# adobe-research/DiffusionHandles

Measured on AMD Instinct MI355X. Metric: guided-denoise steps/sec at 512x512 (SD2-depth), higher is better.
Workload: dtype f16

## Files before the change

### diffusionhandles_amd/_lib.py

```python
import ctypes
import os

import torch

_HERE = os.path.dirname(os.path.abspath(__file__))
LIB_PATH = os.environ.get("DIFFHANDLES_LIB") or os.path.join(_HERE, "libdiffhandles_hip.so")
_LIB = None

c_p = ctypes.c_void_p
c_i = ctypes.c_int
c_f = ctypes.c_float
c_d = ctypes.c_double
c_sz = ctypes.c_size_t


class UNetConfig(ctypes.Structure):
    _fields_ = [("in_channels", c_i), ("out_channels", c_i), ("n_levels", c_i),
                ("block_out_channels", c_i * 4), ("layers_per_block", c_i), ("heads", c_i * 4),
                ("cross_attention_dim", c_i), ("norm_groups", c_i), ("sample_size", c_i),
                ("text_len", c_i), ("max_batch", c_i), ("dtype", c_i), ("max_diff_batch", c_i)]


class VAEConfig(ctypes.Structure):
    _fields_ = [("latent_channels", c_i), ("out_channels", c_i), ("block_out_channels", c_i * 4),
# ... 11 lines not shown
    "dh_device_count": (c_i, []),
    "dh_reproject_workspace_bytes": (c_i, [c_i, c_i, c_i, ctypes.POINTER(c_sz)]),
    "dh_fg_pixel_list": (c_i, [c_p, c_i, c_p, c_p, c_p, c_sz, c_p]),
    "dh_reproject_edits": (c_i, [c_p, c_p, c_p, c_i, c_i, c_p, c_p, c_f, c_f, c_d, c_d, c_i,
                                 ctypes.POINTER(c_d), c_p, c_p, c_p, c_p, c_p, c_p, c_p, c_p, c_p, c_p, c_sz, c_p]),
    "dh_unproject": (c_i, [c_p, c_i, c_p, c_p, c_f, c_f, c_p, c_p]),
    "dh_masked_centroid": (c_i, [c_p, c_p, c_i, c_i, c_p, c_p, c_f, c_f, c_p, c_p]),
    "dh_laplacian_blend_workspace_bytes": (c_i, [c_i, ctypes.POINTER(c_sz)]),
    "dh_laplacian_blend": (c_i, [c_p, c_p, c_p, c_i, c_i, c_p, c_p, c_p, c_sz, c_p]),
    "dh_cells_workspace_bytes": (c_i, [c_i, c_i, ctypes.POINTER(c_sz)]),
    "dh_cells_from_correspondences": (c_i, [c_p, c_i, c_i, c_i, c_i, c_p, c_p, c_p, c_p, c_p, c_sz, c_p]),
    "dh_energy_workspace_bytes": (c_i, [c_i, c_i, c_i, ctypes.POINTER(c_sz)]),
    "dh_energy_fwd_bwd": (c_i, [c_p, c_p, c_i, c_i, c_i, c_i, c_i, c_p, c_i, c_p, c_i, c_p, c_i, c_p, c_i,
                                c_f, c_f, c_i, c_i, c_i, c_f, c_p, c_p, c_i, c_p, c_sz, c_p]),
    "dh_mesh_workspace_bytes": (c_i, [c_i, ctypes.POINTER(c_sz)]),
    "dh_mesh_reproject": (c_i, [c_p, c_p, c_p, c_i, c_p, c_p, c_f, c_f, c_p, c_p, c_f, c_p, c_p, c_p, c_p, c_p, c_p,
                                c_sz, c_p]),
    "dh_energy_plan_bytes": (c_i, [c_i, c_i, ctypes.POINTER(c_sz)]),
    "dh_energy_plan_build": (c_i, [c_p, c_i, c_p, c_i, c_i, c_p, c_sz, c_p]),
    "dh_energy_planned_workspace_bytes": (c_i, [c_i, c_i, ctypes.POINTER(c_sz)]),
    "dh_energy_fwd_bwd_planned": (c_i, [c_p, c_p, c_i, c_i, c_i, c_p, c_sz, c_i, c_p, c_i, c_p, c_i, c_f, c_f, c_f,
                                        c_p, c_p, c_i, c_p, c_sz, c_p]),
    "dh_unet_create": (c_i, [ctypes.POINTER(UNetConfig), ctypes.POINTER(c_p)]),
    "dh_unet_create_shared": (c_i, [c_p, c_i, c_p, ctypes.POINTER(c_p)]),
    "dh_unet_destroy": (None, [c_p]),
    "dh_unet_num_params": (c_i, [c_p]),
    "dh_unet_param_info": (c_i, [c_p, c_i, ctypes.POINTER(ctypes.c_char_p), ctypes.POINTER(c_i),
                                 ctypes.POINTER(ctypes.c_int64)]),
    "dh_unet_load_param": (c_i, [c_p, c_i, c_p, c_p]),
    "dh_unet_weight_bytes": (c_sz, [c_p]),
    "dh_unet_workspace_bytes": (c_sz, [c_p]),
    "dh_unet_forward": (c_i, [c_p, c_p, c_f, c_p, c_i, c_i, c_p, ctypes.POINTER(c_p), c_p]),
    "dh_unet_backward": (c_i, [c_p, ctypes.POINTER(c_p), c_p, c_p, c_p, c_p]),
    "dh_unet_set_text_key": (c_i, [c_p, ctypes.c_ulonglong]),
    "dh_unet_stats": (c_i, [c_p, ctypes.POINTER(c_d), ctypes.POINTER(c_d), ctypes.POINTER(ctypes.c_int64)]),
    "dh_vae_decoder_create": (c_i, [c_p, ctypes.POINTER(c_p)]),
    "dh_vae_decoder_destroy": (None, [c_p]),
    "dh_vae_decoder_num_params": (c_i, [c_p]),
    "dh_vae_decoder_param_info": (c_i, [c_p, c_i, ctypes.POINTER(ctypes.c_char_p), ctypes.POINTER(c_i),
                                        ctypes.POINTER(ctypes.c_int64)]),
    "dh_vae_decoder_load_param": (c_i, [c_p, c_i, c_p, c_p]),
    "dh_vae_decoder_bytes": (c_sz, [c_p]),
    "dh_vae_decoder_decode": (c_i, [c_p, c_p, c_i, c_p, c_p]),
    "dh_vae_encoder_create": (c_i, [c_p, ctypes.POINTER(c_p)]),
    "dh_vae_encoder_encode": (c_i, [c_p, c_p, c_i, c_p, c_p]),
    "dh_text_encoder_create": (c_i, [c_p, ctypes.POINTER(c_p)]),
    "dh_text_encoder_destroy": (None, [c_p]),
    "dh_text_encoder_num_params": (c_i, [c_p]),
    "dh_text_encoder_param_info": (c_i, [c_p, c_i, ctypes.POINTER(ctypes.c_char_p), ctypes.POINTER(c_i),
                                         ctypes.POINTER(ctypes.c_int64)]),
    "dh_text_encoder_load_param": (c_i, [c_p, c_i, c_p, c_p]),
    "dh_text_encoder_bytes": (c_sz, [c_p]),
    "dh_text_encoder_encode": (c_i, [c_p, c_p, c_i, c_i, c_p, c_p]),
    "dh_gemm_profile_begin": (c_i, []),
    "dh_gemm_profile_end": (c_i, [ctypes.POINTER(c_d), ctypes.POINTER(ctypes.c_int64), ctypes.POINTER(c_d)]),
    "dh_gemm_profile_bytes": (c_i, [ctypes.POINTER(c_d)]),
    "dh_ddim_cfg_step": (c_i, [c_p, c_p, c_p, c_p, c_f, c_f, c_f, c_i, c_p]),
    "dh_latent_update": (c_i, [c_p, c_p, c_p, c_f, c_f, c_i, c_p]),
    "dh_adam_step": (c_i, [c_p, c_p, c_p, c_p, c_f, c_f, c_f, c_f, c_i, c_i, c_p]),
    "dh_mse_fwd_bwd": (c_i, [c_p, c_p, c_i, c_p, c_p, c_p]),
    "dh_latent_update_strided": (c_i, [c_p, c_p, c_p, c_i, c_i, c_f, c_f, c_i, c_p]),
    "dh_pack_sample": (c_i, [c_p, c_p, c_i, c_i, c_p, c_i, c_i, c_i, c_i, c_p]),
    "dh_unet_io_ptr": (c_i, [c_p, c_i, c_i, ctypes.POINTER(c_p), ctypes.POINTER(c_sz)]),
    "dh_mse_cotangent": (c_i, [c_p, c_p, c_i, c_f, c_f, c_p, c_p, c_p, c_p]),
    "dh_adam_step_scaled": (c_i, [c_p, c_p, c_p, c_p, c_p, c_f, c_f, c_f, c_f, c_i, c_i, c_p]),
    "dh_mse_cotangent_batch": (c_i, [c_p, c_p, c_i, c_i, c_f, c_f, c_d, c_p, c_p, c_p, c_p, c_p, c_p]),
    "dh_adam_step_scaled_batch": (c_i, [c_p, c_p, c_p, c_p, c_p, c_p, c_f, c_f, c_f, c_f, c_i, c_i, c_i, c_p]),
}

c_l = ctypes.c_long
DEBUG_SIGNATURES = {
    "dh_dbg_gemm": (c_i, [c_i, c_p, c_l, c_p, c_i, c_i, c_i, c_i, c_i, c_i, c_i, c_i, c_i, c_i, c_i, c_p, c_p, c_i, c_i,
                          c_p, c_l, c_p, c_l, c_i, c_p, c_sz, c_p]),
    "dh_dbg_gemm_groupnorm": (c_i, [c_i, c_p, c_l, c_p, c_i, c_i, c_i, c_i, c_i, c_i, c_i, c_p, c_p, c_p, c_sz, c_i, c_i, c_p, c_p, c_f, c_i,
                                    c_p, c_p, c_p, ctypes.POINTER(c_i), c_p]),
    "dh_dbg_gemm_groupnorm_bwd": (c_i, [c_i, c_p, c_l, c_p, c_i, c_i, c_i, c_i, c_i, c_i, c_i, c_p, c_p, c_sz, c_i, c_i, c_p, c_p, c_p, c_p, c_i,
                                        c_p, c_p, ctypes.POINTER(c_i), c_p]),
    "dh_dbg_gemm_groupnorm_res": (c_i, [c_i, c_p, c_l, c_p, c_i, c_i, c_i, c_i, c_i, c_i, c_i, c_p, c_p, c_l, c_p, c_p, c_sz, c_i, c_i, c_p, c_p,
                                    c_f, c_i, c_p, c_p, c_p, ctypes.POINTER(c_i), c_p]),
    "dh_dbg_gemm_groupnorm_bwd_res": (c_i, [c_i, c_p, c_l, c_p, c_i, c_i, c_i, c_i, c_i, c_i, c_i, c_p, c_l, c_p, c_p, c_sz, c_i, c_i, c_p, c_p, c_p,
                                        c_p, c_i, c_p, c_p, ctypes.POINTER(c_i), c_p]),
    "dh_dbg_concat_groupnorm": (c_i, [c_i, c_p, c_i, c_p, c_i, c_p, c_i, c_i, c_i, c_p, c_p, c_f, c_i, c_p, c_p, c_p, c_p]),
    "dh_dbg_gemm_last_tile": (c_i, [ctypes.POINTER(c_i)]),
    "dh_dbg_unet_concat_ops": (c_i, [ctypes.POINTER(UNetConfig), ctypes.POINTER(c_i), c_i, ctypes.POINTER(c_i)]),
    "dh_dbg_gemm_lnfold": (c_i, [c_i, c_p, c_l, c_p, c_i, c_i, c_i, c_p, c_p, c_p, c_f, c_p, c_l, c_p]),
    "dh_dbg_gemm_glu": (c_i, [c_i, c_i, c_p, c_l, c_p, c_i, c_i, c_i, c_p, c_p, c_p, c_p, c_p, c_p]),
    "dh_dbg_gemm_family": (c_i, [c_i]),
    "dh_dbg_gemm_stage": (c_i, [c_i]),
    "dh_dbg_gemm_pp_variant": (c_i, [c_i, c_p]),
    "dh_dbg_gemm_pp_ablate": (c_i, [c_i]),
    "dh_dbg_gemm_pp_persist": (c_i, [c_i]),
    "dh_dbg_gemm_pp_glu": (c_i, [c_i]),
    "dh_dbg_gemm_pp_plan": (c_i, [c_i, c_i, c_i, c_i, c_i, c_i, c_sz, ctypes.POINTER(c_i), ctypes.POINTER(c_i), ctypes.POINTER(c_i)]),
    "dh_dbg_touch_tiled": (c_i, [c_sz, c_p]),
    "dh_dbg_groupnorm": (c_i, [c_i, c_p, c_p, c_p, c_p, c_p, c_p, c_p, c_p, c_i, c_i, c_i, c_i, c_f, c_i, c_i, c_p]),
    "dh_dbg_layernorm": (c_i, [c_i, c_p, c_p, c_p, c_p, c_p, c_p, c_p, c_p, c_i, c_i, c_f, c_p]),
    "dh_dbg_geglu": (c_i, [c_i, c_p, c_p, c_p, c_p, c_i, c_i, c_p]),
    "dh_dbg_attention": (c_i, [c_i, c_p, c_l, c_p, c_p, c_l, c_p, c_l, c_p, c_p, c_p, c_p, c_p, c_p, c_i, c_i, c_i, c_i, c_p]),
    "dh_dbg_attention_bwd_pair": (c_i, [c_i, c_p, c_l, c_p, c_p, c_l, c_p, c_l, c_p, c_p, c_p, c_p, c_p, c_p, c_i, c_i, c_i, c_i, c_p, c_p]),
    "dh_dbg_pool2x2": (c_i, [c_i, c_p, c_p, c_i, c_i, c_i, c_i, c_i, c_p]),
    "dh_dbg_ellipse_offsets": (c_i, [c_i, ctypes.POINTER(ctypes.c_int32), c_i, ctypes.POINTER(c_i)]),
    "dh_dbg_lane_ops": (c_i, [c_p, c_p, c_p, c_p]),
}


def lib():
    global _LIB
    if _LIB is None:
        if not os.path.exists(LIB_PATH):
            raise RuntimeError(
                f"native HIP library not found at {LIB_PATH}; build it with "
                "`python -c 'import __graft_entry__ as g; g.build()'` (there is no CPU fallback)")
        handle = ctypes.CDLL(LIB_PATH)
        missing = []
        for name, (res, args) in list(SIGNATURES.items()) + list(DEBUG_SIGNATURES.items()):
            try:
                fn = getattr(handle, name)
            except AttributeError:
                missing.append(name)
                continue
            fn.restype = res
            fn.argtypes = args
        handle.dh_missing_symbols = missing
        for env, fn in (("DH_GEMM_FAMILY", "dh_dbg_gemm_family"), ("DH_PP_GLU", "dh_dbg_gemm_pp_glu"),
                        ("DH_PP_PERSIST", "dh_dbg_gemm_pp_persist"), ("DH_GEMM_STAGE", "dh_dbg_gemm_stage")):
            if os.environ.get(env) and fn not in missing:
                getattr(handle, fn)(int(os.environ[env]))
        _LIB = handle
    return _LIB


def check(rc, what=""):
    if rc != 0:
        raise RuntimeError(f"{what} failed ({rc}): {lib().dh_last_error().decode()}")


def require_gpu(t=None):
    if not torch.cuda.is_available():
        raise RuntimeError("diffusionhandles_amd needs a HIP device (MI355X); there is no CPU fallback")
    if t is not None and not t.is_cuda:
        raise RuntimeError("expected a device tensor")


def ptr(t):
    return c_p(t.data_ptr()) if t is not None else c_p(0)


def stream_ptr():
    return c_p(torch.cuda.current_stream().cuda_stream)


DTYPE_CODE = {torch.float16: 0, torch.bfloat16: 1, torch.float32: 2}
CODE_DTYPE = {v: k for k, v in DTYPE_CODE.items()}
```

### diffusionhandles_amd/csrc/gemm.hip

```cpp
#include <stdlib.h>

#include <vector>

#include <hip/hip_ext.h>

#include "gemm_k.h"

namespace dh {

struct GemmProf {
  bool on = false;
  std::vector<hipEvent_t> ev;
  size_t used = 0;
  double flops = 0;
  double bytes = 0;
  hipEvent_t e0 = nullptr, e1 = nullptr;
};
static GemmProf g_prof;
static int g_buf_stage = 1;
static int g_pp_force = 0;
struct GemmTileReport {
  int bm, bn, kg, stages, mw, splits, pp, gn_epi, reduce_gn;
};
static thread_local GemmTileReport g_last_tile;
#ifdef DH_TUNING
static unsigned long long* g_gemm_ts = nullptr;
#endif
bool gemm_profiling_on() { return g_prof.on; }

constexpr int BK = 64;
#ifdef DH_EXP_SETPRIO
#define DH_PRIO(x) __builtin_amdgcn_s_setprio(x)
#else
#define DH_PRIO(x) do { } while (0)
#endif


template <class T>
__device__ __forceinline__ uint2 epilogue_pack(const GemmK& p, int m, int n, float v0, float v1, float v2, float v3,
                                               bool have_r, uint2 rpre, bool have_b, float4 bpre) {
  float v[4] = {v0, v1, v2, v3};
  if (p.bias) {
    float4 b = bpre;
    if (!have_b) b = *reinterpret_cast<const float4*>(p.bias + n);
    v[0] += b.x; v[1] += b.y; v[2] += b.z; v[3] += b.w;
  }
  if (p.rowvec) {
    const float4 b = *reinterpret_cast<const float4*>(p.rowvec + (size_t)div_small(m, p.inv_rows_per_batch) * p.rowvec_ld + n);
    v[0] += b.x; v[1] += b.y; v[2] += b.z; v[3] += b.w;
  }
  if (p.act_silu) {
#pragma unroll
    for (int i = 0; i < 4; ++i) v[i] = v[i] / (1.f + __expf(-v[i]));
  }
  typedef T T4 __attribute__((ext_vector_type(4)));
  if (p.R) {
    const T* r = reinterpret_cast<const T*>(p.R) + (size_t)m * p.ldr + n;
    uint2 raw = rpre;
    if (!have_r) raw = *reinterpret_cast<const uint2*>(r);
    const T4 rv = __builtin_bit_cast(T4, raw);
#pragma unroll
    for (int i = 0; i < 4; ++i) v[i] += to_f32<T>(rv[i]);
  }
  T4 o;
#pragma unroll
  for (int i = 0; i < 4; ++i) o[i] = from_f32<T>(v[i]);
  return __builtin_bit_cast(uint2, o);
}
template <class T>
__device__ __forceinline__ void epilogue_store(const GemmK& p, int m, int n, float v0, float v1, float v2, float v3,
                                               bool have_r = false, uint2 rpre = make_uint2(0, 0), bool have_b = false,
                                               float4 bpre = make_float4(0.f, 0.f, 0.f, 0.f)) {
  *reinterpret_cast<uint2*>(reinterpret_cast<T*>(p.C) + (size_t)m * p.ldc + n) =
      epilogue_pack<T>(p, m, n, v0, v1, v2, v3, have_r, rpre, have_b, bpre);
}

template <class T>
__device__ __forceinline__ float epilogue_scalar(const GemmK& p, int m, int n, float v) {
  if (p.bias) v += p.bias[n];
  if (p.rowvec) v += p.rowvec[(size_t)div_small(m, p.inv_rows_per_batch) * p.rowvec_ld + n];
  if (p.act_silu) v = v / (1.f + __expf(-v));
  if (p.R) v += to_f32<T>(reinterpret_cast<const T*>(p.R)[(size_t)m * p.ldr + n]);
  return to_f32<T>(from_f32<T>(v));
}

__device__ uint4 g_zero_page[8];

__device__ __forceinline__ void dma16(const void* gsrc, unsigned lds_dst) {
  unsigned keep;
  asm volatile("s_mov_b32 %0, m0\n\ts_mov_b32 m0, %2\n\ts_nop 0\n\tglobal_load_lds_dwordx4 %1, off\n\ts_mov_b32 m0, %0"
               : "=&s"(keep) : "v"(gsrc), "s"(lds_dst) : "memory");
}

__device__ __forceinline__ void dma16_nt(const void* gsrc, unsigned lds_dst) {
  unsigned keep;
  asm volatile("s_mov_b32 %0, m0\n\ts_mov_b32 m0, %2\n\ts_nop 0\n\tglobal_load_lds_dwordx4 %1, off nt\n\ts_mov_b32 m0, %0"
               : "=&s"(keep) : "v"(gsrc), "s"(lds_dst) : "memory");
}

typedef int buf_v4i __attribute__((ext_vector_type(4)));
__device__ __forceinline__ void buf_dma16(unsigned voff, buf_v4i rsrc, unsigned soff, unsigned lds_dst) {
  unsigned tmp;
  soff = __builtin_amdgcn_readfirstlane(soff);
  lds_dst = __builtin_amdgcn_readfirstlane(lds_dst);
  asm volatile("s_mov_b32 m0, %4\n\ts_mov_b32 %0, %3\n\tbuffer_load_dwordx4 %1, %2, %0 offen lds"
// ... 907 lines not shown
    }
    if (p.act_silu) {
#pragma unroll
      for (int i = 0; i < 8; ++i) v[i] = v[i] / (1.f + __expf(-v[i]));
    }
    if (p.R) {
      const uint4 raw = *reinterpret_cast<const uint4*>(reinterpret_cast<const T*>(p.R) + (size_t)m * p.ldr + n);
      const T* rv = reinterpret_cast<const T*>(&raw);
#pragma unroll
      for (int i = 0; i < 8; ++i) v[i] += to_f32<T>(rv[i]);
    }
    T o[8];
    if (!BWD) {
#pragma unroll
      for (int i = 0; i < 8; ++i) { o[i] = from_f32<T>(v[i]); f[i] = to_f32<T>(o[i]); }
    } else {
      const uint4 rawx = *reinterpret_cast<const uint4*>(reinterpret_cast<const T*>(p.gnb_x) + (size_t)m * p.gnb_ldx + n);
      const T* xv = reinterpret_cast<const T*>(&rawx);
#pragma unroll
      for (int i = 0; i < 8; ++i) {
        o[i] = from_f32<T>(v[i]);
        const float xh = (to_f32<T>(xv[i]) - mu[i]) * rs[i];
        float d = to_f32<T>(o[i]);
        if (p.gnb_silu) d *= silu_grad(xh * gm[i] + bt[i]);
        d *= gm[i];
        av[i] += d; qv[i] += d * xh;
      }
    }
    *reinterpret_cast<uint4*>(reinterpret_cast<T*>(p.C) + (size_t)m * p.ldc + n) = *reinterpret_cast<uint4*>(o);
  };
  auto acc = [&](const float* f) {
#pragma unroll
    for (int i = 0; i < 8; ++i) { const float d = f[i] - pv[i]; av[i] += d; qv[i] += d * d; }
  };
  float f[8];
  if (BWD) {
    if (live)
      for (int r = r0 + rr; r < r1; r += RP) row(r, f);
  } else {
    const bool first = live && r0 + rr < r1;
    if (first) row(r0 + rr, f);
    if (first && rr == 0) {
#pragma unroll
      for (int i = 0; i < 8; ++i)
        if (ch * 8 + i == gi[i] * cpg) sm_piv[gi[i]] = f[i];
    }
    __syncthreads();
#pragma unroll
    for (int i = 0; i < 8; ++i) pv[i] = g0 + gi[i] < G ? sm_piv[gi[i]] : 0.f;
    if (first) {
      acc(f);
      for (int r = r0 + rr + RP; r < r1; r += RP) { row(r, f); acc(f); }
    }
  }
  if (live) {
#pragma unroll
    for (int i = 0; i < 8; ++i)
#pragma unroll
      for (int gl = 0; gl < GN_GB; ++gl) {
        ga[gl] += gi[i] == gl ? av[i] : 0.f;
        gq[gl] += gi[i] == gl ? qv[i] : 0.f;
      }
  }
#pragma unroll
  for (int gl = 0; gl < GN_GB; ++gl) { ga[gl] = wave_sum(ga[gl]); gq[gl] = wave_sum(gq[gl]); }
  if ((threadIdx.x & 63) == 0) {
#pragma unroll
    for (int gl = 0; gl < GN_GB; ++gl) { sm_red[threadIdx.x >> 6][2 * gl] = ga[gl]; sm_red[threadIdx.x >> 6][2 * gl + 1] = gq[gl]; }
  }
  __syncthreads();
  if ((int)threadIdx.x < GN_GB && g0 + (int)threadIdx.x < G) {
    const int gl = threadIdx.x, g = g0 + gl;
    float sa = 0.f, sq = 0.f;
    for (int w = 0; w < 4; ++w) { sa += sm_red[w][2 * gl]; sq += sm_red[w][2 * gl + 1]; }
    if (BWD) {
      p.gn_part[((size_t)(b * G + g) * S + s) * 2] = sa;
      p.gn_part[((size_t)(b * G + g) * S + s) * 2 + 1] = sq;
    } else {
      const float cnt = (float)(r1 - r0) * (float)cpg;
      float* o = p.gn_part + ((size_t)(b * G + g) * 3) * S + s;
      o[0] = cnt; o[S] = sm_piv[gl] + sa / cnt; o[2 * S] = sq - sa * sa / cnt;
    }
  }
}

#define DH_GEMM_LAUNCH(KERNEL)                                                                              \
  do {                                                                                                      \
    if (g_prof.e0) hipExtLaunchKernelGGL(KERNEL, grid, dim3(TH), 0, st, g_prof.e0, g_prof.e1, 0, k);        \
    else hipLaunchKernelGGL(KERNEL, grid, dim3(TH), 0, st, k);                                              \
  } while (0)
template <class T, int BM, int BN, int ST, int WG, int KG, int MW, bool BUF>
static void launch_tile_b(int gm, bool lnf, dim3 grid, hipStream_t st, const GemmK& k, int glu) {
  constexpr int TH = 256 * WG * KG * MW;
  constexpr bool GLUOK = WG == 1 && KG == 1 && ((BM == 256 && BN == 128 && MW == 2) || (BM == 128 && BN == 128 && MW == 2 && ST == 4) || (BM == 64 && BN == 64));
  if constexpr (GLUOK) {
    if (glu == 1 && lnf) { DH_GEMM_LAUNCH((k_gemm_dma<T, BM, BN, ST, GM_DENSE, 0, WG, KG, MW, true, 1, BUF>)); return; }
    if (glu == 1) { DH_GEMM_LAUNCH((k_gemm_dma<T, BM, BN, ST, GM_DENSE, 0, WG, KG, MW, false, 1, BUF>)); return; }
    if (glu == 2) { DH_GEMM_LAUNCH((k_gemm_dma<T, BM, BN, ST, GM_DENSE, 0, WG, KG, MW, false, 2, BUF>)); return; }
  }
  if (gm == GM_DENSE) {
    if constexpr (WG == 1 && BN != 320 && BN != 160) {
      if (lnf) { DH_GEMM_LAUNCH((k_gemm_dma<T, BM, BN, ST, GM_DENSE, 0, WG, KG, MW, true, 0, BUF>)); return; }
    }
    DH_GEMM_LAUNCH((k_gemm_dma<T, BM, BN, ST, GM_DENSE, 0, WG, KG, MW, false, 0, BUF>));
  } else if (gm == GM_CONV_S1) {
    DH_GEMM_LAUNCH((k_gemm_dma<T, BM, BN, ST, GM_CONV_S1, 0, WG, KG, MW, false, 0, BUF>));
  } else {
    DH_GEMM_LAUNCH((k_gemm_dma<T, BM, BN, ST, GM_GENERIC, 0, WG, KG, MW>));
  }
}
template <class T, int BM, int BN, int ST, int WG, int KG, int MW>
static void launch_tile(int gm, bool lnf, dim3 grid, hipStream_t st, const GemmK& k, int glu = 0) {
  g_last_tile.bm = BM; g_last_tile.bn = BN; g_last_tile.kg = KG; g_last_tile.stages = ST; g_last_tile.mw = MW;
  if (k.pp_a_bytes != 0 && gm != GM_GENERIC) launch_tile_b<T, BM, BN, ST, WG, KG, MW, true>(gm, lnf, grid, st, k, glu);
  else launch_tile_b<T, BM, BN, ST, WG, KG, MW, false>(gm, lnf, grid, st, k, glu);
}
#undef DH_GEMM_LAUNCH

#ifdef DH_TUNING
#define DH_KNOB(name, env, dflt) static const int name = getenv(env) ? atoi(getenv(env)) : (dflt)
#else
#define DH_KNOB(name, env, dflt) constexpr int name = (dflt)
#endif

template <class T>
static void gemm_dispatch(GemmK k, size_t partial_elems, hipStream_t st, int* gn_done, int* lnb_done, int dtype) {
  DH_KNOB(kSplitTiles, "DH_SPLITK_TILES", 200);
  DH_KNOB(kSplitMinK, "DH_SPLITK_MINKT", 32);
  DH_KNOB(kSplitTarget, "DH_SPLITK_TARGET", 256);
  DH_KNOB(kBigTiles, "DH_BIG_TILES", 128);
  DH_KNOB(kNarrowTiles, "DH_NARROW_TILES", 40);
  DH_KNOB(kN320, "DH_GEMM_N320", 224);
  DH_KNOB(kMwBlocks, "DH_GEMM_MW", 64);
  DH_KNOB(kKg2MinKt, "DH_KG2_MINKT", 4);
  DH_KNOB(kManyBlocks, "DH_GEMM_MANY", 512);
  DH_KNOB(kMw128, "DH_GEMM_MW128", 1);
  DH_KNOB(kTwoPerCu, "DH_GEMM_TWO_PER_CU", 1);
#ifdef DH_TUNING
  DH_KNOB(kWnt, "DH_W_NT", 0);
#endif
  const bool lnf = k.ln_s != nullptr;
  g_last_tile = GemmTileReport{};
  int BM = 128, BN = (k.N % 128 == 0) ? 128 : 64;
  const int ktiles = k.K / BK;
  PpPlan pp;
  const bool use_pp = gemm_pp_plan(k, partial_elems, g_pp_force, &pp);
  if (BN == 128 && ktiles >= 16 && cdiv(k.M, 128) * cdiv(k.N, 128) <= kNarrowTiles) BN = 64;
  if (k.M <= 64 || (cdiv(k.M, 128) * cdiv(k.N, BN) < kBigTiles && ktiles < kSplitMinK)) { BM = 64; BN = 64; }
  const bool n320 = kN320 > 0 && k.N % 320 == 0 && k.N <= 960 && !lnf && BM == 128 && BN == 64 && cdiv(k.M, 128) >= kN320;
  if (n320) BN = 320;
  DH_KNOB(kMwShortK, "DH_GEMM_MW_SHORTK", 128);
  const long tiles256 = (long)cdiv(k.M, 256) * cdiv(k.N, 128);
  const bool mw2 = kMwBlocks > 0 && k.N % 128 == 0 && tiles256 >= kMwBlocks &&
                   !(k.M <= 256 && k.M > 128 && cdiv(k.N, 128) < 128) && (tiles256 >= kMwShortK || ktiles >= kSplitMinK);
  if (mw2) { BM = 256; BN = 128; }
  const int glu = k.glu_y ? 1 : (k.glub_x ? 2 : 0);
  if (glu && !(BM == 64 && BN == 64)) { BM = mw2 ? 256 : 128; BN = 128; }
  DH_KNOB(kT160, "DH_GEMM_T160", 224);
  const long tiles160 = (long)cdiv(k.M, 128) * (k.N / 160);
  const bool t160 = kT160 > 0 && k.N % 160 == 0 && !lnf && !glu && !n320 && BM != 64 && tiles160 >= kT160 && tiles160 <= 256;
  if (t160) { BM = 128; BN = 160; }
  if (use_pp) { BM = pp.bm; BN = pp.bn; }
  const int tm = cdiv(k.M, BM), tn = cdiv(k.N, BN), tiles = tm * tn;
  int splits = 1;
  if (use_pp) splits = pp.splits;
  else if (k.partial && !lnf && !glu && tiles < kSplitTiles && ktiles >= kSplitMinK) {
    splits = kSplitTarget / tiles;
    if (splits > ktiles / 4) splits = ktiles / 4;
    if (splits > 32) splits = 32;
    const size_t fit = partial_elems / ((size_t)k.M * k.N);
    if ((size_t)splits > fit) splits = (int)fit;
    if (splits < 1) splits = 1;
  }
#ifdef DH_TUNING
  static const int kLog = getenv("DH_GEMM_LOG") ? atoi(getenv("DH_GEMM_LOG")) : 0;
  const int kForceTile = getenv("DH_FORCE_TILE") ? atoi(getenv("DH_FORCE_TILE")) : 0;
  const int kForceSplits = getenv("DH_FORCE_SPLITS") ? atoi(getenv("DH_FORCE_SPLITS")) : 0;
  int force_tile = 0;
  if (kForceTile && !use_pp && !(k.glu_y || k.glub_x)) {
    const int fbm = kForceTile == 1 ? 64 : (kForceTile == 6 ? 256 : 128), fbn = kForceTile == 7 ? 160 : ((kForceTile <= 3) ? 64 : 128);
    if ((k.N % fbn == 0 || fbn == 64) && !(fbn == 160 && lnf)) { BM = fbm; BN = fbn; force_tile = kForceTile; }
  }
  if (kForceSplits && !use_pp && k.partial && !lnf) {
    splits = kForceSplits;
    if (splits > ktiles / 2) splits = ktiles / 2 > 0 ? ktiles / 2 : 1;
    const size_t fit = partial_elems / ((size_t)k.M * k.N);
    if ((size_t)splits > fit) splits = (int)fit;
    if (splits < 1) splits = 1;
  }
  if (kLog) fprintf(stderr, "GEMMLOG M=%d N=%d K=%d mode=%d lnf=%d gn=%d gnb=%d bias=%d R=%d rowvec=%d | pp=%d BM=%d BN=%d splits=%d\n", k.M, k.N, k.K,
                    k.mode == A_DENSE ? 0 : (k.mode == A_CONV3 && k.stride == 1 && k.up == 0 ? 1 : 2), (int)lnf, k.gn_part != nullptr,
                    k.gnb_x != nullptr, k.bias != nullptr, k.R != nullptr, k.rowvec != nullptr, (int)use_pp, BM, BN, splits);
#endif
  const int tiles_per_split = cdiv(ktiles, splits);
  splits = cdiv(ktiles, tiles_per_split);
  k.splits = splits;
  k.k_per_split = tiles_per_split * BK;
  k.gn_epi = 0; k.gn_cpg = 0;
  if ((g_buf_stage & 4) == 0 && splits == 1 && !use_pp && gn_epi_fwd_tile(BN, glu, lnf) && k.gn_part && !k.gnb_x && gn_done && k.gn_G > 0 &&
      k.gn_HW > 0 && k.C && k.wide_store && k.M % k.gn_HW == 0 && k.gn_HW % BM == 0 && k.N % k.gn_G == 0 && k.N % BN == 0) {
    const int cpg = k.N / k.gn_G, sx = 2 * (k.gn_HW / BM);
    if (cpg >= 8 && cpg <= BN && sx <= 64) { k.gn_epi = 1; k.gn_cpg = cpg; k.gn_S = sx; }
  }
  if ((g_buf_stage & 8) == 0 && splits == 1 && !use_pp && gn_epi_bwd_tile(BM, BN, 1, glu, lnf) && k.gn_part && k.gnb_x && gn_done && k.gn_G > 0 &&
      k.gn_HW > 0 && k.C && k.wide_store && k.pre_r && !k.R && !k.bias && !k.rowvec && !k.act_silu && k.M % k.gn_HW == 0 && k.gn_HW % BM == 0 &&
      k.N % k.gn_G == 0 && k.N % BN == 0 && (((size_t)k.gnb_x | (size_t)(k.gnb_ldx * 2)) & 7) == 0) {
    const int cpg = k.N / k.gn_G, sx = 2 * (k.gn_HW / BM);
    if (cpg >= 8 && cpg <= BN && sx <= 64) { k.gn_epi = 2; k.gn_cpg = cpg; k.gn_S = sx; }
  }
#ifdef DH_TUNING
  k.w_nt = kWnt > 0 && tm <= kWnt;
  static const int kLnfAbl = getenv("DH_LNF_ABL") ? atoi(getenv("DH_LNF_ABL")) : 0;
  k.lnf_abl = kLnfAbl;
  k.ts = g_gemm_ts;
#endif
#ifdef DH_TUNING
  dim3 grid(force_tile ? cdiv(k.M, BM) : tm, force_tile ? cdiv(k.N, BN) : tn, splits);
#else
  dim3 grid(tm, tn, splits);
#endif
  hipEvent_t e0 = nullptr, e1 = nullptr;
  if (g_prof.on) {
    if (g_prof.used + 2 > g_prof.ev.size()) {
      const size_t old = g_prof.ev.size();
      g_prof.ev.resize(old + 4096);
      for (size_t i = old; i < g_prof.ev.size(); ++i) (void)hipEventCreate(&g_prof.ev[i]);
    }
    e0 = g_prof.ev[g_prof.used++];
    e1 = g_prof.ev[g_prof.used++];
    g_prof.flops += 2.0 * (double)k.M * (double)k.N * (double)k.K;
    const double esz = 2.0;
    double a_elems = (double)k.M * k.K;
    if (k.mode != A_DENSE && k.Hout > 0 && k.Wout > 0) a_elems = (double)k.M / ((double)k.Hout * k.Wout) * k.Hin * k.Win * k.Cin;
    double c_elems = (double)k.M * k.N * (k.C ? 1.0 : 0.0) + (k.R ? (double)k.M * k.N : 0.0);
    if (k.glu_y) c_elems += 0.5 * (double)k.M * k.N;
    if (k.glub_x) c_elems += 4.0 * (double)k.M * k.N;
    if (k.gn_epi == 2) c_elems += (double)k.M * k.N;
    g_prof.bytes += esz * (a_elems + (double)k.N * k.K + c_elems);
    g_prof.e0 = e0; g_prof.e1 = e1;
  }
  int gm = GM_GENERIC;
  if (k.mode == A_DENSE) gm = GM_DENSE;
  else if (k.mode == A_CONV3 && k.stride == 1 && k.up == 0 && k.pad == 1) gm = GM_CONV_S1;
  if (!use_pp) {
    k.pp_a_bytes = 0; k.pp_w_bytes = 0;
    size_t ab = 0;
    if (k.mode == A_DENSE) ab = ((size_t)(k.M - 1) * k.lda + k.K) * 2;
    else if (k.Hout > 0 && k.Wout > 0 && k.M % (k.Hout * k.Wout) == 0)
      ab = (size_t)(k.M / (k.Hout * k.Wout)) * k.Hin * k.Win * (size_t)k.lda * 2;
    const size_t wb = (size_t)align_up((size_t)k.N, 64) * k.K * 2;
    const bool conv_ok = k.mode == A_DENSE || (k.Cin % 64 == 0 && k.K == 9 * k.Cin);
    if ((g_buf_stage & 1) && ab > 0 && conv_ok && ab + (size_t)(k.Win + 1) * k.lda * 2 < 0x7ff00000ull && wb < 0x7ff00000ull && k.lda % 8 == 0 &&
        ((size_t)k.A & 15) == 0 && ((size_t)k.W & 15) == 0) {
      k.pp_a_bytes = (unsigned)ab; k.pp_w_bytes = (unsigned)wb;
    }
  }
#ifdef DH_TUNING
  static const int kAbl = getenv("DH_GEMM_ABLATE") ? atoi(getenv("DH_GEMM_ABLATE")) : 0;
  if (kAbl == 1 && BM == 128 && BN == 128) { hipLaunchKernelGGL((k_gemm_dma<T, 128, 128, 4, GM_CONV_S1, 1>), grid, dim3(256), 0, st, k); }
  else if (kAbl == 2 && BM == 128 && BN == 128) { hipLaunchKernelGGL((k_gemm_dma<T, 128, 128, 4, GM_CONV_S1, 2>), grid, dim3(256), 0, st, k); }
  else if (kAbl == 3 && BM == 128 && BN == 128) { hipLaunchKernelGGL((k_gemm_dma<T, 128, 128, 4, GM_DENSE, 1>), grid, dim3(256), 0, st, k); }
  else if (kAbl == 1 && mw2 && gm == GM_CONV_S1) { hipLaunchKernelGGL((k_gemm_dma<T, 256, 128, 3, GM_CONV_S1, 1, 1, 1, 2>), grid, dim3(512), 0, st, k); }
  else if (kAbl == 2 && mw2 && gm == GM_CONV_S1) { hipLaunchKernelGGL((k_gemm_dma<T, 256, 128, 3, GM_CONV_S1, 2, 1, 1, 2>), grid, dim3(512), 0, st, k); }
  else if (kAbl == 1 && mw2 && gm == GM_DENSE && !lnf) { hipLaunchKernelGGL((k_gemm_dma<T, 256, 128, 3, GM_DENSE, 1, 1, 1, 2>), grid, dim3(512), 0, st, k); }
  else if (kAbl == 2 && mw2 && gm == GM_DENSE && !lnf) { hipLaunchKernelGGL((k_gemm_dma<T, 256, 128, 3, GM_DENSE, 2, 1, 1, 2>), grid, dim3(512), 0, st, k); }
  else if (force_tile == 1) launch_tile<T, 64, 64, 4, 1, 1, 1>(gm, lnf, grid, st, k);
  else if (force_tile == 2) launch_tile<T, 128, 64, 3, 1, 2, 1>(gm, lnf, grid, st, k);
  else if (force_tile == 3) launch_tile<T, 128, 64, 5, 1, 1, 1>(gm, lnf, grid, st, k);
  else if (force_tile == 4) launch_tile<T, 128, 128, 4, 1, 1, 2>(gm, lnf, grid, st, k);
  else if (force_tile == 5) launch_tile<T, 128, 128, 4, 1, 1, 1>(gm, lnf, grid, st, k);
  else if (force_tile == 6) launch_tile<T, 256, 128, 3, 1, 1, 2>(gm, lnf, grid, st, k);
  else if (force_tile == 7) launch_tile<T, 128, 160, 4, 1, 1, 1>(gm, false, grid, st, k);
  else
#endif
  if (use_pp) { pp.splits = splits; g_last_tile.bm = pp.bm; g_last_tile.bn = pp.bn; launch_gemm_pp(dtype, k, pp, st, g_prof.e0, g_prof.e1); }
  else if (t160) launch_tile<T, 128, 160, 4, 1, 1, 1>(gm, false, grid, st, k);
  else if (mw2) launch_tile<T, 256, 128, 3, 1, 1, 2>(gm, lnf, grid, st, k, glu);
  else if (BM == 128 && BN == 128 && (glu || (kMw128 && tiles_per_split >= kMw128))) launch_tile<T, 128, 128, 4, 1, 1, 2>(gm, lnf, grid, st, k, glu);
  else if (kTwoPerCu && BM == 128 && BN == 64 && tiles * splits > 256 && tiles * splits <= 512)
    launch_tile<T, 128, 64, 3, 1, 1, 1>(gm, lnf, grid, st, k);
  else if (BM == 128 && BN == 64 && tiles_per_split >= kKg2MinKt) launch_tile<T, 128, 64, 3, 1, 2, 1>(gm, lnf, grid, st, k);
  else if (BN == 320) launch_tile<T, 128, 320, 2, 1, 1, 2>(gm, false, grid, st, k);
  else if (BM == 64) launch_tile<T, 64, 64, 4, 1, 1, 1>(gm, lnf, grid, st, k, glu);
  else if (BN == 128 && kManyBlocks > 0 && tiles * splits >= kManyBlocks) launch_tile<T, 128, 128, 2, 1, 1, 1>(gm, lnf, grid, st, k);
  else if (BN == 128) launch_tile<T, 128, 128, 4, 1, 1, 1>(gm, lnf, grid, st, k);
  else launch_tile<T, 128, 64, 5, 1, 1, 1>(gm, lnf, grid, st, k);
  g_prof.e0 = g_prof.e1 = nullptr;
  g_last_tile.splits = splits; g_last_tile.pp = use_pp ? 1 : 0; g_last_tile.gn_epi = k.gn_epi;
  if (k.gn_epi) *gn_done = k.gn_S;
  if (splits > 1) {
    if (k.gn_part && k.gn_G > 0 && k.gn_HW > 0 && k.N % k.gn_G == 0 && (GN_GB * (k.N / k.gn_G)) % 8 == 0 &&
        GN_GB * (k.N / k.gn_G) <= 2048 && k.M % k.gn_HW == 0) {
      k.gn_S = gn_slices(k.gn_HW, k.M / k.gn_HW);
      if (k.gnb_x) hipLaunchKernelGGL((k_splitk_reduce_gn<T, true>), dim3(k.gn_S, cdiv(k.gn_G, GN_GB), k.M / k.gn_HW), dim3(256), 0, st, k);
      else hipLaunchKernelGGL((k_splitk_reduce_gn<T, false>), dim3(k.gn_S, cdiv(k.gn_G, GN_GB), k.M / k.gn_HW), dim3(256), 0, st, k);
      g_last_tile.reduce_gn = 1;
      if (gn_done) *gn_done = 1;
    } else if (k.lnb_x && lnb_done && !k.bias && !k.rowvec && !k.R && !k.act_silu && k.N % 8 == 0 && k.ldc == k.N) {
      launch_splitk_reduce_ln_bwd(dtype, k.partial, splits, k.lnb_x, k.lnb_gamma, k.lnb_stats, k.lnb_add, k.lnb_dx, k.M, k.N, st);
      *lnb_done = 1;
    } else {
      const size_t groups = (size_t)k.M * k.N / 4;
      hipLaunchKernelGGL((k_splitk_reduce<T>), dim3((unsigned)((groups + 255) / 256)), dim3(256), 0, st, k);
    }
  }
}
#undef DH_KNOB

double launch_gemm(int dtype, const GemmArgs& a, hipStream_t st) {
  GemmK k;
  k.A = a.A; k.lda = a.lda; k.W = a.W; k.M = a.M; k.N = a.N; k.K = a.K;
  k.mode = a.mode; k.Hin = a.Hin; k.Win = a.Win; k.Cin = a.Cin; k.Hout = a.Hout; k.Wout = a.Wout;
  k.stride = a.stride; k.up = a.up; k.pad = a.pad;
  k.bias = a.bias; k.rowvec = a.rowvec; k.rowvec_ld = a.rowvec_ld;
  k.rows_per_batch = a.rows_per_batch > 0 ? a.rows_per_batch : 1;
  k.inv_rows_per_batch = 1.f / (float)k.rows_per_batch;
  k.R = a.R; k.ldr = a.ldr; k.C = a.C; k.ldc = a.ldc; k.act_silu = a.act_silu;
  k.partial = a.partial; k.splits = 1; k.k_per_split = a.K;
  k.pre_r = 1;
  k.wide_store = a.N % 32 == 0 && a.ldc % 8 == 0 && ((size_t)a.C & 15) == 0;
  k.ln_s = a.ln_s; k.ln_t = a.ln_t; k.ln_stats = a.ln_stats; k.ln_eps = a.ln_eps;
  k.gn_part = a.gn_part; k.gn_HW = a.gn_HW; k.gn_G = a.gn_G; k.gn_S = 0;
  k.gnb_x = a.gnb_x; k.gnb_ldx = a.gnb_ldx; k.gnb_gamma = a.gnb_gamma; k.gnb_beta = a.gnb_beta; k.gnb_stats = a.gnb_stats;
  k.gnb_silu = a.gnb_silu;
  k.lnb_x = a.lnb_x; k.lnb_gamma = a.lnb_gamma; k.lnb_stats = a.lnb_stats; k.lnb_add = a.lnb_add; k.lnb_dx = a.lnb_dx;
  k.glu_y = a.glu_y; k.glu_ldy = a.glu_ldy; k.glub_x = a.glub_x; k.glub_dx = a.glub_dx;
  if (a.gn_done) *a.gn_done = 0;
  if (a.lnb_done) *a.lnb_done = 0;
  if (dtype == DH_DTYPE_F16) gemm_dispatch<f16>(k, a.partial_elems, st, a.gn_done, a.lnb_done, dtype);
  else gemm_dispatch<bf16>(k, a.partial_elems, st, a.gn_done, a.lnb_done, dtype);
  return 2.0 * (double)a.M * (double)a.N * (double)a.K;
}

}

#ifdef DH_TUNING
extern "C" int dh_dbg_gemm_timeline(unsigned long long* ts) { dh::g_gemm_ts = ts; return DH_OK; }
#endif

extern "C" int dh_dbg_gemm_family(int force) {
  DH_REQUIRE(force >= 0 && force <= 2, "family: 0 policy, 1 k_gemm_dma, 2 k_gemm_pp");
  dh::g_pp_force = force;
  return DH_OK;
}

extern "C" int dh_dbg_gemm_stage(int buf) {
  dh::g_buf_stage = buf;
  return DH_OK;
}

extern "C" int dh_dbg_gemm_last_tile(int* out) {
  DH_REQUIRE(out != nullptr, "null pointer");
  const dh::GemmTileReport& r = dh::g_last_tile;
  const int v[9] = {r.bm, r.bn, r.kg, r.stages, r.mw, r.splits, r.pp, r.gn_epi, r.reduce_gn};
  for (int i = 0; i < 9; ++i) out[i] = v[i];
  return DH_OK;
}

extern "C" int dh_gemm_profile_begin(void) {
  dh::g_prof.on = true;
  dh::g_prof.used = 0;
  dh::g_prof.flops = 0;
  dh::g_prof.bytes = 0;
  return DH_OK;
}
extern "C" int dh_gemm_profile_bytes(double* bytes) {
  if (bytes) *bytes = dh::g_prof.bytes;
  return DH_OK;
}
extern "C" int dh_gemm_profile_end(double* ms_total, int64_t* launches, double* flops) {
  using namespace dh;
  g_prof.on = false;
  double ms = 0;
  if (g_prof.used >= 2) DH_CHECK_HIP(hipEventSynchronize(g_prof.ev[g_prof.used - 1]));
  for (size_t i = 0; i + 1 < g_prof.used; i += 2) {
    float t = 0;
    DH_CHECK_HIP(hipEventElapsedTime(&t, g_prof.ev[i], g_prof.ev[i + 1]));
    ms += t;
  }
  if (ms_total) *ms_total = ms;
  if (launches) *launches = (int64_t)(g_prof.used / 2);
  if (flops) *flops = g_prof.flops;
  return DH_OK;
}
```

Before: 36.41.

## Add slab-resident split-K implicit-GEMM kernel for small 3x3 convolutions

Adds a dedicated split-K kernel for stride-1 3x3 convolutions on 16x16 and 8x8 feature maps with large weight tensors. Each block loads a whole image's row slab for a 64-channel chunk into LDS once and reuses it across all nine taps, while weights stream through a three-deep DMA ring with dynamic vmcnt waits. The aim is to remove redundant im2col activation loads and expose more parallelism on the low-resolution UNet convs, which are weight-bandwidth bound. The cost is larger LDS use per block and new dispatch logic that overrides the policy's split count, plus a debug query reporting when the new path was taken.

```diff
diff --git a/diffusionhandles_amd/_lib.py b/diffusionhandles_amd/_lib.py
--- a/diffusionhandles_amd/_lib.py
+++ b/diffusionhandles_amd/_lib.py
@@ -117,6 +117,7 @@
                                         c_p, c_i, c_p, c_p, ctypes.POINTER(c_i), c_p]),
     "dh_dbg_concat_groupnorm": (c_i, [c_i, c_p, c_i, c_p, c_i, c_p, c_i, c_i, c_i, c_p, c_p, c_f, c_i, c_p, c_p, c_p, c_p]),
     "dh_dbg_gemm_last_tile": (c_i, [ctypes.POINTER(c_i)]),
+    "dh_dbg_gemm_last_tile_ex": (c_i, [ctypes.POINTER(c_i), c_i]),
     "dh_dbg_unet_concat_ops": (c_i, [ctypes.POINTER(UNetConfig), ctypes.POINTER(c_i), c_i, ctypes.POINTER(c_i)]),
     "dh_dbg_gemm_lnfold": (c_i, [c_i, c_p, c_l, c_p, c_i, c_i, c_i, c_p, c_p, c_p, c_f, c_p, c_l, c_p]),
     "dh_dbg_gemm_glu": (c_i, [c_i, c_i, c_p, c_l, c_p, c_i, c_i, c_i, c_p, c_p, c_p, c_p, c_p, c_p]),
diff --git a/diffusionhandles_amd/csrc/gemm.hip b/diffusionhandles_amd/csrc/gemm.hip
--- a/diffusionhandles_amd/csrc/gemm.hip
+++ b/diffusionhandles_amd/csrc/gemm.hip
@@ -20,7 +20,7 @@
 static int g_buf_stage = 1;
 static int g_pp_force = 0;
 struct GemmTileReport {
-  int bm, bn, kg, stages, mw, splits, pp, gn_epi, reduce_gn;
+  int bm, bn, kg, stages, mw, splits, pp, gn_epi, reduce_gn, slab;
 };
 static thread_local GemmTileReport g_last_tile;
 #ifdef DH_TUNING
@@ -1094,6 +1094,187 @@
       o[0] = cnt; o[S] = sm_piv[gl] + sa / cnt; o[2 * S] = sq - sa * sa / cnt;
     }
   }
+}
+
+constexpr int SL_WR = 3;
+constexpr int SL_WT = 8192;
+
+template <int LO, int HI> __device__ __forceinline__ void wait_vmcnt_dyn(int n) {
+  if constexpr (LO == HI) { wait_vmcnt<LO>(); }
+  else {
+    constexpr int MID = (LO + HI + 1) / 2;
+    if (n >= MID) wait_vmcnt_dyn<MID, HI>(n); else wait_vmcnt_dyn<LO, MID - 1>(n);
+  }
+}
+
+template <class T, int BM, int SLABR>
+__global__ void __launch_bounds__(64 * (BM / 32 > 4 ? BM / 32 : 4)) k_conv_slab_s(const GemmK p) {
+  constexpr int WMS = BM / 32, NWV = WMS > 4 ? WMS : 4, WNS = NWV / WMS;
+  constexpr int CPW = 64 / WNS, TN = CPW / 32;
+  constexpr int NPW = 8 / NWV;
+  constexpr int NPL = (SLABR / 8 + NWV - 1) / NWV;
+  constexpr int SLAB = SLABR * 128, RING = 2 * SLAB, ZERO = RING + SL_WR * 3 * SL_WT, LDS = ZERO + 128;
+  static_assert(BM % 32 == 0 && WNS * WMS == NWV && TN >= 1 && NPW * NWV == 8, "wave layout");
+  static_assert(SLABR % 8 == 0 && LDS <= 160 * 1024 && NPL <= 9 && NPL * NWV * 8 >= SLABR, "slab layout");
+  __shared__ __attribute__((aligned(1024))) unsigned char smem[LDS];
+  const int tid = threadIdx.x, lane = tid & 63;
+  const int wave = __builtin_amdgcn_readfirstlane(tid >> 6);
+  const int wm = wave / WNS, wn = wave - wm * WNS, ln = lane & 31, hi = lane >> 5;
+  const int Wimg = p.Win, HW = p.Hin * p.Win;
+  const int m0 = blockIdx.x * BM, n0 = blockIdx.y * 64;
+  const int b = m0 / HW, p0 = m0 - b * HW;
+  const int chunks = p.Cin >> 6, cps = p.k_per_split / 576;
+  const int cbeg = blockIdx.z * cps;
+  const int cend = cbeg + cps < chunks ? cbeg + cps : chunks;
+  const int nsteps = (cend - cbeg) * 3;
+  const unsigned lds0 = (unsigned)(size_t)((__attribute__((address_space(3))) unsigned char*)smem);
+
+  if (tid < 32) reinterpret_cast<unsigned*>(smem + ZERO)[tid] = 0u;
+  __syncthreads();
+
+  buf_v4i ra, rw;
+  ra[0] = (int)(unsigned)(size_t)p.A; ra[1] = (int)(((size_t)p.A >> 32) & 0xffff); ra[2] = (int)p.pp_a_bytes; ra[3] = 0x00020000;
+  rw[0] = (int)(unsigned)(size_t)p.W; rw[1] = (int)(((size_t)p.W >> 32) & 0xffff); rw[2] = (int)p.pp_w_bytes; rw[3] = 0x00020000;
+  const int rows_needed = BM + 2 * Wimg + 2;
+  unsigned sv[NPL];
+#pragma unroll
+  for (int k = 0; k < NPL; ++k) {
+    const int s = (wave + NWV * k) * 8 + (lane >> 3);
+    const int q = p0 - Wimg - 1 + s;
+    const bool ok = s < rows_needed && q >= 0 && q < HW;
+    const int lchunk = (lane & 7) ^ ((s >> 1) & 7);
+    sv[k] = ok ? (unsigned)(b * HW + q) * (unsigned)((int)p.lda * 2) + (unsigned)lchunk * 16u : 0x80000000u;
+  }
+  const int npieces = (rows_needed + 7) >> 3;
+  const unsigned wv = (unsigned)(wave * NPW) * 1024u + lane * 16u;
+  const unsigned wbase = (unsigned)((n0 >> 6) * (p.K >> 6)) * (unsigned)SL_WT + (unsigned)cbeg * 9u * (unsigned)SL_WT;
+  int issued = 0;
+  auto issue_slab_piece = [&](int c, int buf, int k) {
+    if (wave + NWV * k < npieces) {
+      buf_dma16(sv[k], ra, (unsigned)c * 128u, lds0 + buf * SLAB + (wave + NWV * k) * 1024);
+      ++issued;
+    }
+  };
+  auto issue_w = [&](int S) {
+    const unsigned dst = lds0 + RING + (S % SL_WR) * (3 * SL_WT) + wave * NPW * 1024;
+#pragma unroll
+    for (int kx = 0; kx < 3; ++kx)
+#pragma unroll
+      for (int j = 0; j < NPW; ++j) buf_dma16(wv + j * 1024, rw, wbase + (unsigned)(3 * S + kx) * SL_WT, dst + kx * SL_WT + j * 1024);
+    issued += 3 * NPW;
+  };
+  int mk[SL_WR - 1];
+#pragma unroll
+  for (int k = 0; k < NPL; ++k) issue_slab_piece(cbeg, 0, k);
+#pragma unroll
+  for (int i = 0; i < SL_WR - 1; ++i) {
+    if (i < nsteps) issue_w(i);
+    mk[i] = issued;
+  }
+  int slab_mk = 0;
+
+  unsigned fb[4];
+#pragma unroll
+  for (int kk = 0; kk < 4; ++kk) fb[kk] = (unsigned)((wn * CPW + ln) * 128) + (unsigned)(((2 * kk + hi) ^ ((ln >> 1) & 7)) << 4);
+  const int r = wm * 32 + ln;
+  const int x = (p0 + r) % Wimg;
+  const bool xl = x == 0, xr = x == Wimg - 1;
+  v16f acc[TN];
+#pragma unroll
+  for (int j = 0; j < TN; ++j)
+#pragma unroll
+    for (int e = 0; e < 16; ++e) acc[j][e] = 0.f;
+
+  int c = 0, ky = 0;
+  for (int S = 0; S < nsteps; ++S) {
+    const int need = ky == 0 && S > 0 && slab_mk > mk[0] ? slab_mk : mk[0];
+    wait_vmcnt_dyn<0, 31>(issued - need);
+    __builtin_amdgcn_s_barrier();
+#pragma unroll
+    for (int i = 0; i < SL_WR - 2; ++i) mk[i] = mk[i + 1];
+    if (S + SL_WR - 1 < nsteps) issue_w(S + SL_WR - 1);
+    mk[SL_WR - 2] = issued;
+    if (ky == 0 && c + 1 < cend - cbeg) {
+#pragma unroll
+      for (int k = 0; k < NPL; ++k) issue_slab_piece(cbeg + c + 1, (c + 1) & 1, k);
+      slab_mk = issued;
+    }
+    unsigned ab[3], sw[3];
+#pragma unroll
+    for (int kx = 0; kx < 3; ++kx) {
+      const int s2 = r + ky * Wimg + kx;
+      const bool z = (kx == 0 && xl) || (kx == 2 && xr);
+      ab[kx] = z ? (unsigned)ZERO : (unsigned)((c & 1) * SLAB + s2 * 128);
+      sw[kx] = z ? 0u : (unsigned)((s2 >> 1) & 7);
+    }
+    const unsigned wt = (unsigned)(RING + (S % SL_WR) * (3 * SL_WT));
+    uint4 fw[2][TN], fx[2];
+    auto load_frags = [&](int q, int bf) {
+      const int kx = q >> 2, kk = q & 3;
+#pragma unroll
+      for (int j = 0; j < TN; ++j) fw[bf][j] = *reinterpret_cast<const uint4*>(smem + wt + kx * SL_WT + fb[kk] + j * (32 * 128));
+      fx[bf] = *reinterpret_cast<const uint4*>(smem + ab[kx] + ((((unsigned)(2 * kk + hi)) ^ sw[kx]) << 4));
+    };
+    load_frags(0, 0);
+#pragma unroll
+    for (int q = 0; q < 12; ++q) {
+      if (q + 1 < 12) load_frags(q + 1, (q + 1) & 1);
+#pragma unroll
+      for (int j = 0; j < TN; ++j) acc[j] = Mfma<T>::run(fw[q & 1][j], fx[q & 1], acc[j]);
+    }
+    if (++ky == 3) { ky = 0; ++c; }
+  }
+
+  const int m = m0 + r;
+#pragma unroll
+  for (int j = 0; j < TN; ++j)
+#pragma unroll
+    for (int g = 0; g < 4; ++g) {
+      const int n = n0 + wn * CPW + j * 32 + 8 * g + 4 * hi;
+      *reinterpret_cast<float4*>(p.partial + ((size_t)blockIdx.z * p.M + m) * p.N + n) =
+          make_float4(acc[j][4 * g], acc[j][4 * g + 1], acc[j][4 * g + 2], acc[j][4 * g + 3]);
+    }
+}
+
+static int conv_slab_s_splits(const GemmK& k, size_t partial_elems, int policy_splits, int target) {
+  if ((g_buf_stage & 16) || policy_splits < 2) return 0;
+  if (!(k.mode == A_CONV3 && k.stride == 1 && k.up == 0 && k.pad == 1) || k.ln_s || k.glu_y || k.glub_x || !k.partial) return 0;
+  if (k.Hin != k.Hout || k.Win != k.Wout || k.Hin != k.Win || (k.Hin != 16 && k.Hin != 8)) return 0;
+  const int HW = k.Hin * k.Win;
+  if (k.M % HW || k.N % 64 || k.Cin % 64 || k.K != 9 * k.Cin || k.lda % 8 || k.lda < k.Cin) return 0;
+  if (((size_t)k.A & 15) || ((size_t)k.W & 15) || ((size_t)k.partial & 15)) return 0;
+  const size_t ab = (size_t)k.M * (size_t)k.lda * 2, wb = (size_t)k.N * k.K * 2;
+  if (ab >= 0x7ff00000ull || wb >= 0x7ff00000ull) return 0;
+  if (wb < (16u << 20)) return 0;
+  const int chunks = k.Cin / 64, tiles = (k.M / HW) * (k.N / 64);
+  int s = target / tiles;
+  if (s > chunks) s = chunks;
+  if (s > 32) s = 32;
+  const size_t fit = partial_elems / ((size_t)k.M * k.N);
+  if ((size_t)s > fit) s = (int)fit;
+  if (s < 2) return 0;
+  const int cps = cdiv(chunks, s);
+  s = cdiv(chunks, cps);
+  return s >= 2 ? s : 0;
+}
+
+template <class T>
+static void launch_conv_slab_s(GemmK& k, int splits, hipStream_t st) {
+  const int chunks = k.Cin / 64, cps = cdiv(chunks, splits), HW = k.Hin * k.Win;
+  k.splits = splits;
+  k.k_per_split = cps * 576;
+  k.pp_a_bytes = (unsigned)((size_t)k.M * (size_t)k.lda * 2);
+  k.pp_w_bytes = (unsigned)((size_t)k.N * k.K * 2);
+  const dim3 grid(k.M / HW, k.N / 64, splits);
+#define DH_SL_LAUNCH(KERNEL, TH)                                                                       \
+  do {                                                                                                 \
+    if (g_prof.e0) hipExtLaunchKernelGGL(KERNEL, grid, dim3(TH), 0, st, g_prof.e0, g_prof.e1, 0, k);   \
+    else hipLaunchKernelGGL(KERNEL, grid, dim3(TH), 0, st, k);                                         \
+  } while (0)
+  if (HW == 256) DH_SL_LAUNCH((k_conv_slab_s<T, 256, 296>), 512);
+  else DH_SL_LAUNCH((k_conv_slab_s<T, 64, 88>), 256);
+#undef DH_SL_LAUNCH
+  g_last_tile.bm = HW; g_last_tile.bn = 64; g_last_tile.kg = 1; g_last_tile.stages = SL_WR; g_last_tile.mw = 1; g_last_tile.slab = 1;
 }
 
 #define DH_GEMM_LAUNCH(KERNEL)                                                                              \
@@ -1204,8 +1385,13 @@
                     k.mode == A_DENSE ? 0 : (k.mode == A_CONV3 && k.stride == 1 && k.up == 0 ? 1 : 2), (int)lnf, k.gn_part != nullptr,
                     k.gnb_x != nullptr, k.bias != nullptr, k.R != nullptr, k.rowvec != nullptr, (int)use_pp, BM, BN, splits);
 #endif
+  int slab_splits = use_pp ? 0 : conv_slab_s_splits(k, partial_elems, splits, kSplitTarget);
+#ifdef DH_TUNING
+  if (force_tile || kForceSplits) slab_splits = 0;
+#endif
+  if (slab_splits) splits = slab_splits;
   const int tiles_per_split = cdiv(ktiles, splits);
-  splits = cdiv(ktiles, tiles_per_split);
+  if (!slab_splits) splits = cdiv(ktiles, tiles_per_split);
   k.splits = splits;
   k.k_per_split = tiles_per_split * BK;
   k.gn_epi = 0; k.gn_cpg = 0;
@@ -1285,7 +1471,8 @@
   else if (force_tile == 7) launch_tile<T, 128, 160, 4, 1, 1, 1>(gm, false, grid, st, k);
   else
 #endif
-  if (use_pp) { pp.splits = splits; g_last_tile.bm = pp.bm; g_last_tile.bn = pp.bn; launch_gemm_pp(dtype, k, pp, st, g_prof.e0, g_prof.e1); }
+  if (slab_splits) launch_conv_slab_s<T>(k, slab_splits, st);
+  else if (use_pp) { pp.splits = splits; g_last_tile.bm = pp.bm; g_last_tile.bn = pp.bn; launch_gemm_pp(dtype, k, pp, st, g_prof.e0, g_prof.e1); }
   else if (t160) launch_tile<T, 128, 160, 4, 1, 1, 1>(gm, false, grid, st, k);
   else if (mw2) launch_tile<T, 256, 128, 3, 1, 1, 2>(gm, lnf, grid, st, k, glu);
   else if (BM == 128 && BN == 128 && (glu || (kMw128 && tiles_per_split >= kMw128))) launch_tile<T, 128, 128, 4, 1, 1, 2>(gm, lnf, grid, st, k, glu);
@@ -1361,6 +1548,13 @@
   return DH_OK;
 }
 
+extern "C" int dh_dbg_gemm_last_tile_ex(int* out, int n) {
+  DH_REQUIRE(out != nullptr && n >= 0, "bad arguments");
+  const dh::GemmTileReport& r = dh::g_last_tile;
+  const int v[10] = {r.bm, r.bn, r.kg, r.stages, r.mw, r.splits, r.pp, r.gn_epi, r.reduce_gn, r.slab};
+  for (int i = 0; i < n && i < 10; ++i) out[i] = v[i];
+  return DH_OK;
+}
 extern "C" int dh_dbg_gemm_last_tile(int* out) {
   DH_REQUIRE(out != nullptr, "null pointer");
   const dh::GemmTileReport& r = dh::g_last_tile;
```

Result: no change. 36.70, median of 6 (+0.8%).
